# Merricx/zksnake

Measured on AMD Instinct MI355X. Metric: BN254 G1 MSM throughput, higher is better.
Workload: dtype u32 limbs (254-bit modular integers)

## Files before the change

zksnake_amd/csrc/msm_reduce.hip.h:

```cpp
#pragma once
#include "msm_common.hip.h"
#include "msm_reduce_plan.h"

namespace zkmi {

constexpr int COMBINE_THREADS = 256;
constexpr uint32_t COMBINE_WAVE_BLOCKS = 128, COMBINE_BIG_BLOCKS = 64;

template <class G>
__global__ __launch_bounds__(COMBINE_THREADS) void combine_kernel(const uint32_t* __restrict__ partials,
                                                                  const uint32_t* __restrict__ run_start, uint32_t n_keys,
                                                                  uint32_t small_blocks, const uint32_t* __restrict__ big_list,
                                                                  const uint32_t* __restrict__ big_count,
                                                                  uint32_t* __restrict__ buckets) {
    typedef typename G::F F;
    constexpr int XW = 4 * F::LIMBS;
    constexpr int HW = HalfRegs<F>::COUNT;
    __shared__ uint32_t sh[COMBINE_THREADS * HW];
    const bool odd = (threadIdx.x & 1) != 0;
    if (blockIdx.x < small_blocks) {
        const uint32_t key = (blockIdx.x * COMBINE_THREADS + threadIdx.x) >> 1;
        if (key >= n_keys) return;
        const uint32_t s0 = run_start[key], s1 = run_start[key + 1];
        if (s1 - s0 == 1 || s1 - s0 > COMBINE_SMALL_MAX) return;
        HalfPt<F> acc = half_inf<F>();
        if (s1 > s0) {
            acc = half_load<F>(partials + (size_t)s0 * XW, odd);
            HalfPt<F> cur = s0 + 1 < s1 ? half_load<F>(partials + (size_t)(s0 + 1) * XW, odd) : half_inf<F>();
            for (uint32_t r = s0 + 1; r < s1; ++r) {
                HalfPt<F> nxt = r + 1 < s1 ? half_load<F>(partials + (size_t)(r + 1) * XW, odd) : half_inf<F>();
                acc = pair_add<F>(acc, cur, odd);
                cur = nxt;
            }
        }
        half_store<F>(buckets + (size_t)key * XW, odd, acc);
    } else if (blockIdx.x < small_blocks + COMBINE_WAVE_BLOCKS) {
        const uint32_t count = big_count[0];
        const uint32_t lane = threadIdx.x & 63, pair = lane >> 1;
        const uint32_t wave = ((blockIdx.x - small_blocks) * COMBINE_THREADS + threadIdx.x) >> 6;
        const uint32_t n_waves = (COMBINE_WAVE_BLOCKS * COMBINE_THREADS) >> 6;
        for (uint32_t b = wave; b < count; b += n_waves) {
            const uint32_t key = big_list[b];
            const uint32_t s0 = run_start[key], s1 = run_start[key + 1];
            HalfPt<F> v = half_inf<F>();
            for (uint32_t r = s0 + pair; r < s1; r += 32) v = pair_add<F>(v, half_load<F>(partials + (size_t)r * XW, odd), odd);
            for (int m = 32; m >= 2; m >>= 1) v = pair_add<F>(v, half_shfl_xor<F>(v, m), odd);
            if (lane < 2) half_store<F>(buckets + (size_t)key * XW, odd, v);
        }
    } else {
        const uint32_t count = big_count[1];
        const uint32_t j = threadIdx.x, pair = j >> 1;
        for (uint32_t b = blockIdx.x - small_blocks - COMBINE_WAVE_BLOCKS; b < count; b += COMBINE_BIG_BLOCKS) {
            const uint32_t key = big_list[n_keys - 1 - b];
            const uint32_t s0 = run_start[key], s1 = run_start[key + 1];
            HalfPt<F> v = half_inf<F>();
            for (uint32_t r = s0 + pair; r < s1; r += COMBINE_THREADS / 2) v = pair_add<F>(v, half_load<F>(partials + (size_t)r * XW, odd), odd);
            for (uint32_t off = COMBINE_THREADS / 4; off >= 1; off >>= 1) {
                half_lds_put<F>(sh, COMBINE_THREADS, j, v);
                __syncthreads();
                if (pair < off) v = pair_add<F>(v, half_lds_get<F>(sh, COMBINE_THREADS, j + 2 * off), odd);
                __syncthreads();
            }
            if (j < 2) half_store<F>(buckets + (size_t)key * XW, odd, v);
        }
    }
}


template <class G>
__global__ __launch_bounds__(256) void strided_sum_kernel(const uint32_t* __restrict__ in, uint32_t* __restrict__ out,
                                                          SumJob j0, SumJob j1, uint32_t lpo) {
    typedef typename G::F F;
    constexpr int XW = 4 * F::LIMBS;
    const uint32_t gid = blockIdx.x * blockDim.x + threadIdx.x;
    uint32_t o = gid / lpo;
    const uint32_t sub = gid % lpo;
    const bool odd = (sub & 1) != 0;
    const uint32_t pair = sub >> 1, n_pairs = lpo >> 1;
    SumJob job = j0;
    if (o >= j0.n_out) {
        o -= j0.n_out;
        job = j1;
    }
    const bool live = o < job.n_out;
    const uint32_t x = live ? o % job.per_group : 0;
    size_t base = live ? (size_t)job.in_offset + (size_t)(o / job.per_group) * job.group_stride + (size_t)(x / job.split) * job.outer + (size_t)(x % job.split) * job.outer2 : 0;
    HalfPt<F> acc = half_inf<F>();
    if (live && pair < job.count) {
        HalfPt<F> cur = half_load<F>(in + (base + (size_t)pair * job.inner) * XW, odd);
        for (uint32_t j = pair; j < job.count; j += n_pairs) {
            const uint32_t jn = j + n_pairs < job.count ? j + n_pairs : j;
            HalfPt<F> nxt = half_load<F>(in + (base + (size_t)jn * job.inner) * XW, odd);
            acc = pair_add<F>(acc, cur, odd);
            cur = nxt;
        }
    }
    for (uint32_t m = lpo >> 1; m >= 2; m >>= 1) {
        HalfPt<F> other = half_shfl_xor<F>(acc, (int)m);
        acc = pair_add<F>(acc, other, odd);
    }
    if (live && sub < 2) half_store<F>(out + ((size_t)job.out_offset + o) * XW, odd, acc);
}

constexpr int HS_THREADS = 2 * WS_BLOCK;
template <class G>
__global__ __launch_bounds__(HS_THREADS) void weighted_sum_kernel(const uint32_t* __restrict__ in0, uint32_t m0, uint32_t n0,
                                                                  const uint32_t* __restrict__ in1, uint32_t m1,
                                                                  uint32_t* __restrict__ out) {
    typedef typename G::F F;
    constexpr int XW = 4 * F::LIMBS;
    extern __shared__ uint32_t sh[];
    const uint32_t tid = threadIdx.x, pj = tid >> 1;
    const bool odd = (tid & 1) != 0;
    const uint32_t bpa0 = (m0 + WS_BLOCK - 1) / WS_BLOCK, bpa1 = (m1 + WS_BLOCK - 1) / WS_BLOCK;
    const bool first = blockIdx.x < n0 * bpa0;
    const uint32_t rel = first ? blockIdx.x : blockIdx.x - n0 * bpa0;
    const uint32_t bpa = first ? bpa0 : bpa1, ma = first ? m0 : m1;
    const uint32_t arr_i = rel / bpa, blk = rel % bpa;
    const uint32_t m = min((uint32_t)WS_BLOCK, ma - blk * WS_BLOCK);
    const uint32_t* arr = (first ? in0 : in1) + ((size_t)arr_i * ma + (size_t)blk * WS_BLOCK) * XW;
    HalfPt<F> v = pj < m ? half_load<F>(arr + (size_t)pj * XW, odd) : half_inf<F>();
    for (uint32_t off = 1; off < m; off <<= 1) {
        half_lds_put<F>(sh, HS_THREADS, tid, v);
        __syncthreads();
        if (pj + off < m) {
            HalfPt<F> o = half_lds_get<F>(sh, HS_THREADS, tid + 2 * off);
            v = pair_add<F>(v, o, odd);
        }
        __syncthreads();
    }
    if (pj == 0) half_store<F>(out + ((size_t)blockIdx.x * 2 + 1) * XW, odd, v);
    if (pj == 0 || pj >= m) v = half_inf<F>();
    uint32_t top = 1;
    while (top < m) top <<= 1;
    for (uint32_t off = top / 2; off >= 1; off >>= 1) {
        half_lds_put<F>(sh, HS_THREADS, tid, v);
        __syncthreads();
        if (pj < off) {
            HalfPt<F> o = half_lds_get<F>(sh, HS_THREADS, tid + 2 * off);
            v = pair_add<F>(v, o, odd);
        }
        __syncthreads();
    }
    if (pj == 0) half_store<F>(out + (size_t)blockIdx.x * 2 * XW, odd, v);
}


template <class G>
inline void launch_combine(const uint32_t* partials, const uint32_t* run_start, uint32_t n_keys, const uint32_t* big_list,
                           const uint32_t* big_count, uint32_t* buckets, hipStream_t st) {
    const uint32_t small_blocks = (2 * n_keys + COMBINE_THREADS - 1) / COMBINE_THREADS;
    hipLaunchKernelGGL(combine_kernel<G>, dim3(small_blocks + COMBINE_WAVE_BLOCKS + COMBINE_BIG_BLOCKS), dim3(COMBINE_THREADS), 0, st,
                       partials, run_start, n_keys, small_blocks, big_list, big_count, buckets);
}

template <class G>
inline void launch_strided_sum(const uint32_t* in, uint32_t* out, const SumJob& j0, const SumJob& j1, uint32_t lpo, hipStream_t st) {
    hipLaunchKernelGGL(strided_sum_kernel<G>, dim3((unsigned)((((uint64_t)j0.n_out + j1.n_out) * lpo + 255) / 256)), dim3(256), 0, st,
                       in, out, j0, j1, lpo);
}

template <class G>
inline hipError_t weighted_sum_set_attributes() {
    return hipFuncSetAttribute((const void*)weighted_sum_kernel<G>, hipFuncAttributeMaxDynamicSharedMemorySize,
                               (int)(HalfRegs<typename G::F>::COUNT * HS_THREADS * 4));
}

template <class G>
inline void launch_weighted_sum(const uint32_t* in0, uint32_t m0, uint32_t n0, const uint32_t* in1, uint32_t m1, uint32_t* out, hipStream_t st) {
    const uint32_t blocks = n0 * ((m0 + WS_BLOCK - 1) / WS_BLOCK + (m1 + WS_BLOCK - 1) / WS_BLOCK);
    hipLaunchKernelGGL(weighted_sum_kernel<G>, dim3(blocks), dim3(HS_THREADS), (size_t)HalfRegs<typename G::F>::COUNT * HS_THREADS * 4, st,
                       in0, m0, n0, in1, m1, out);
}

}
```

Measured before the change: 696.8.

## Compact long small-bucket runs into a block-local queue to reduce divergence

In the small-key path of the combine kernel, every thread pair now does its first pairwise add directly. Runs of length 2 are stored immediately and empty runs get an infinity store. Keys with more than two partials are pushed into a shared-memory queue via an LDS atomic, then repacked onto the leading lanes so the remaining serial adds run on densely packed waves. This targets wave divergence when run lengths vary, in exchange for extra barriers, LDS traffic and a DPP lane broadcast.

```diff
diff --git a/zksnake_amd/csrc/msm_reduce.hip.h b/zksnake_amd/csrc/msm_reduce.hip.h
--- a/zksnake_amd/csrc/msm_reduce.hip.h
+++ b/zksnake_amd/csrc/msm_reduce.hip.h
@@ -19,21 +19,49 @@
     __shared__ uint32_t sh[COMBINE_THREADS * HW];
     const bool odd = (threadIdx.x & 1) != 0;
     if (blockIdx.x < small_blocks) {
+        __shared__ uint32_t q_count, q_key[COMBINE_THREADS / 2], q_next[COMBINE_THREADS / 2], q_left[COMBINE_THREADS / 2];
+        if (threadIdx.x == 0) q_count = 0;
         const uint32_t key = (blockIdx.x * COMBINE_THREADS + threadIdx.x) >> 1;
-        if (key >= n_keys) return;
-        const uint32_t s0 = run_start[key], s1 = run_start[key + 1];
-        if (s1 - s0 == 1 || s1 - s0 > COMBINE_SMALL_MAX) return;
-        HalfPt<F> acc = half_inf<F>();
-        if (s1 > s0) {
-            acc = half_load<F>(partials + (size_t)s0 * XW, odd);
-            HalfPt<F> cur = s0 + 1 < s1 ? half_load<F>(partials + (size_t)(s0 + 1) * XW, odd) : half_inf<F>();
-            for (uint32_t r = s0 + 1; r < s1; ++r) {
-                HalfPt<F> nxt = r + 1 < s1 ? half_load<F>(partials + (size_t)(r + 1) * XW, odd) : half_inf<F>();
-                acc = pair_add<F>(acc, cur, odd);
-                cur = nxt;
+        uint32_t s0 = 0, runs = 1;
+        if (key < n_keys) {
+            s0 = run_start[key];
+            runs = run_start[key + 1] - s0;
+        }
+        __syncthreads();
+        if (runs == 0) {
+            half_store<F>(buckets + (size_t)key * XW, odd, half_inf<F>());
+        } else if (runs >= 2 && runs <= COMBINE_SMALL_MAX) {
+            const HalfPt<F> r0 = half_load<F>(partials + (size_t)s0 * XW, odd);
+            const HalfPt<F> r1 = half_load<F>(partials + (size_t)(s0 + 1) * XW, odd);
+            const HalfPt<F> acc = pair_add<F>(r0, r1, odd);
+            if (runs == 2) {
+                half_store<F>(buckets + (size_t)key * XW, odd, acc);
+            } else {
+                uint32_t e = odd ? 0u : atomicAdd(&q_count, 1u);
+                const uint32_t e_even = (uint32_t)__builtin_amdgcn_mov_dpp((int)e, 0xB1, 0xF, 0xF, true);
+                if (odd) e = e_even;
+                half_lds_put<F>(sh, COMBINE_THREADS, 2 * e + (odd ? 1u : 0u), acc);
+                if (!odd) {
+                    q_key[e] = key;
+                    q_next[e] = s0 + 2;
+                    q_left[e] = runs - 2;
+                }
             }
         }
-        half_store<F>(buckets + (size_t)key * XW, odd, acc);
+        __syncthreads();
+        const uint32_t e = threadIdx.x >> 1;
+        if (e >= q_count) return;
+        const uint32_t q_k = q_key[e];
+        uint32_t r = q_next[e], left = q_left[e];
+        HalfPt<F> cur = half_load<F>(partials + (size_t)r * XW, odd);
+        HalfPt<F> acc = half_lds_get<F>(sh, COMBINE_THREADS, threadIdx.x);
+        for (; left != 0; --left) {
+            ++r;
+            HalfPt<F> nxt = left > 1 ? half_load<F>(partials + (size_t)r * XW, odd) : half_inf<F>();
+            acc = pair_add<F>(acc, cur, odd);
+            cur = nxt;
+        }
+        half_store<F>(buckets + (size_t)q_k * XW, odd, acc);
     } else if (blockIdx.x < small_blocks + COMBINE_WAVE_BLOCKS) {
         const uint32_t count = big_count[0];
         const uint32_t lane = threadIdx.x & 63, pair = lane >> 1;
```

Measured after the change: 700.3, median of 5. About the same (+0.5%).
